# gue-ni/raytracer.c

Hardware: AMD Instinct MI355X
Metric: ray-bounces/sec (higher is better)
Workload: dtype f64

## Files before the change

raytracer.c_amd/csrc/pt_body_pooled.h:

```cpp
#ifndef PT_BODY_POOLED_H
#define PT_BODY_POOLED_H


#ifndef PT_MIN_WAVES
#define PT_MIN_WAVES 5
#endif
#ifndef PT_MIN_WAVES_TRI
#define PT_MIN_WAVES_TRI 5
#endif
#ifndef PT_MIN_WAVES_CHK
#define PT_MIN_WAVES_CHK 5
#endif
#ifndef PT_MESH_BATCH
#define PT_MESH_BATCH 32
#endif
#ifndef PT_MESH_MAX_WAIT
#define PT_MESH_MAX_WAIT 16
#endif
#ifndef PT_DIR_ROUNDS
#define PT_DIR_ROUNDS 4
#endif
#ifndef PT_DIR_MIN_LANES
#define PT_DIR_MIN_LANES 1
#endif
template <bool CHECKER, bool TRIS, bool FILT_LDS, bool GEOM_LDS, bool REFR = false>
__device__ __forceinline__ void render_tiles_pooled(const PtLaunch &L, const bool LIST)
{
  static_assert(!REFR || (CHECKER && FILT_LDS && (GEOM_LDS || !TRIS)), "the pooled refraction kernels: sphere scenes (staged, or streamed from memory) and small staged mesh scenes, every material");
  extern __shared__ __attribute__((aligned(16))) double lds[];
  __shared__ float out_f[PT_TILE_PIXELS * 3];
  __shared__ uint8_t out_b[PT_TILE_PIXELS * 3 + 64];
  __shared__ unsigned long long wg_stats[2];
  __shared__ double cam_lds[PT_CAM_LDS_DOUBLES];
  __shared__ unsigned long long pix_sum[REFR ? 1 : PT_TILE_PIXELS * 3];
  __shared__ unsigned long long pix_win[REFR ? PT_TILE_PIXELS * 3 * PT_WIN_N : 1];
  __shared__ unsigned long long pend_free[REFR ? PT_BLOCK / 64 : 1][2];
  __shared__ uint32_t pend_slot_lds;
  __shared__ unsigned long long pix_nan[3];
  __shared__ unsigned long long pix_key[PT_TILE_PIXELS];
  constexpr bool DEFER_MESH = TRIS && !FILT_LDS;
  constexpr bool SWAP = !DEFER_MESH;
  __shared__ double q_dir[SWAP ? 1 : PT_BLOCK / 64][SWAP ? 1 : 3 * 64];
  __shared__ unsigned long long q_rng[SWAP ? 1 : PT_BLOCK / 64][SWAP ? 1 : 64];
  __shared__ uint32_t q_pix[SWAP ? 1 : PT_BLOCK / 64][SWAP ? 1 : 64];
  constexpr uint32_t WAIT_F = CHECKER ? 11u : 10u;
  __shared__ double w_f[SWAP ? PT_BLOCK / 64 : 1][SWAP ? WAIT_F : 1][SWAP ? 64 : 1];
  __shared__ uint32_t w_u[SWAP ? PT_BLOCK / 64 : 1][SWAP ? 2 : 1][SWAP ? 64 : 1];
  constexpr uint32_t CULL_WORDS = GEOM_LDS ? PT_FILT_LDS_MAX / 64 : 256u;
  __shared__ uint32_t tile_pairs[CULL_WORDS];
  __shared__ uint32_t wg_next_job;

#ifdef PT_PHASE
  if ((threadIdx.x & 63u) == 0u)
  {
    for (int k = 0; k < PT_PHASE_SLOTS; k++)
      pt_phase_acc[threadIdx.x >> 6][k] = 0;
    pt_phase_last[threadIdx.x >> 6] = __builtin_amdgcn_s_memtime();
  }
#endif
  SceneCtx S_init = stage_scene<GEOM_LDS, FILT_LDS>(L, lds);
  __shared__ double atan_tab[CHECKER ? PT_ATAN_TAB : 1];
  if (CHECKER)
  {
    atan_table_to_lds(atan_tab);
    S_init.atan_tab = atan_tab;
  }
  PHASE(8);
  __shared__ __attribute__((aligned(16))) float big_tab[12];
  if (SWAP && FILT_LDS && !TRIS && L.big_pairs != 0u)
  {
    if (threadIdx.x < 2 + 2 * PT_BIG_PAIRS)
      big_tab[threadIdx.x] = threadIdx.x == 0 ? L.big_delta : (threadIdx.x == 1 ? L.big_tmin : L.big_qmin[threadIdx.x - 2]);
    S_init.big = BigPrune{big_tab, L.big_pairs};
  }
  const SceneCtx S = S_init;
  if (threadIdx.x < 2)
    wg_stats[threadIdx.x] = 0;
  if (threadIdx.x == 2)
    wg_next_job = 0;
  if (threadIdx.x < 3)
    pix_nan[threadIdx.x] = 0;
  if (!REFR && threadIdx.x < PT_TILE_PIXELS * 3)
    pix_sum[threadIdx.x] = 0;
  if (REFR)
  {
    for (uint32_t k = threadIdx.x; k < PT_TILE_PIXELS * 3 * PT_WIN_N; k += PT_BLOCK)
      pix_win[k] = 0;
    if (threadIdx.x < 2 * (PT_BLOCK / 64))
      pend_free[threadIdx.x >> 1][threadIdx.x & 1u] = ~0ull;
    if (threadIdx.x == 0)
      pend_slot_lds = pt_pool_acquire(L.pend_flags, L.pend_slots_per_xcd, L.status, PT_FAIL_PEND_SLOT);
  }
  if (threadIdx.x < PT_TILE_PIXELS)
  {
    const uint32_t t0 = L.tile_first + launch_slot(L, blockIdx.x % launch_slots(L, LIST), LIST) * L.tile_stride;
    const uint32_t kx = (t0 % L.tiles_x) * PT_TILE + (threadIdx.x & 7u), ky = (t0 / L.tiles_x) * PT_TILE + (threadIdx.x >> 3);
    pix_key[threadIdx.x] = rt_rng_pixel_key(L.seed, ky * (uint32_t)L.width + kx);
  }
  camera_to_lds(L, cam_lds);
  PHASE(9);
  __syncthreads();
  PHASE(10);

  const uint32_t wave = threadIdx.x >> 6;
  const uint32_t slot = launch_slot(L, blockIdx.x % launch_slots(L, LIST), LIST), chunk = blockIdx.x / launch_slots(L, LIST);
  const uint32_t tile = L.tile_first + slot * L.tile_stride;
  const bool cull_ok = S.n_sph + S.n_tri <= 64u * CULL_WORDS;
  if (SWAP && FILT_LDS && cull_ok)
  {
    tile_cull(cam_lds, L.scene.entry_src, S.n_sph, S.n_sph + S.n_tri, (tile % L.tiles_x) * PT_TILE, (tile / L.tiles_x) * PT_TILE, tile_pairs);
    __syncthreads();
  }
  const uint32_t tx0 = (tile % L.tiles_x) * PT_TILE, ty0 = (tile / L.tiles_x) * PT_TILE + (SWAP ? 0u : 2u * wave);
  const uint32_t vcols = min((uint32_t)PT_TILE, (uint32_t)L.width - tx0);
  const uint32_t vrows = ty0 >= (uint32_t)L.height ? 0u : min(SWAP ? (uint32_t)PT_TILE : 2u, (uint32_t)L.height - ty0);
  const uint32_t n_valid = vcols * vrows;
  const uint32_t spp = (uint32_t)L.samples;
  const uint32_t s_begin = L.sample_first + (uint32_t)(((uint64_t)chunk * spp) / L.sample_chunks);
  const uint32_t s_end = L.sample_first + (uint32_t)(((uint64_t)(chunk + 1u) * spp) / L.sample_chunks);
  const uint32_t pool_jobs = n_valid * (s_end - s_begin);

  Path P;
  P.o = {0, 0, 0};
  P.d = {0, 0, 1};
  P.T = {1, 1, 1};
  P.Ls = {0, 0, 0};
  P.rng = 1;
  P.depth = 0;
  uint32_t n_rays = 0, n_casts = 0;
  constexpr bool PARK_T = TRIS && FILT_LDS && !CHECKER;
  __shared__ double t_park[PARK_T ? 3 : 1][PARK_T ? PT_BLOCK : 1];
  HitRec hit;
  hit.min_t = 0;
  hit.bary_u = 0;
  hit.bary_v = 0;
  hit.best = -1;
  hit.depth_ok = false;
  hit.need_dir = false;
  hit.dir_slot = 0;
  hit.dir_scale = 1.0;
  hit.last.idx = -1;
  hit.last.u = 0;
  hit.last.v = 0;
  bool mesh_wait = false;
  uint32_t trip = 0, wait_since = 0xFFFFFFFFu;
  uint32_t next_job = 0;
  uint32_t made_jobs = 0;
  uint32_t pix_slot = 0;
  bool busy = false;
  int stack_n = 0;
  uint32_t pend_id = 0xFFu;
  const PendStack no_stack = {nullptr, 0, 0u, 0u};
  const uint32_t pend_slot = REFR ? pend_slot_lds : 0u;
  const bool pend_ok = !REFR || pend_slot != 0xFFFFFFFFu;
  const uint32_t pool = pend_ok ? pool_jobs : 0u;
  double *const pend_wave = REFR && pend_ok ? L.pend_ws + (size_t)pend_slot * L.pend_slot_doubles +
                                                  (size_t)(threadIdx.x >> 6) * 128u * L.pend_entries * PT_PEND_FIELDS
                                            : nullptr;
  unsigned long long *diag_ptr = L.stats;
  (void)diag_ptr;
  const uint32_t lane = threadIdx.x & 63u;
  double *const qd = q_dir[wave];
  unsigned long long *const qr = q_rng[wave];
  uint32_t *const qp = q_pix[wave];

  uint32_t n_wait = 0;
  double *const wf = &w_f[SWAP ? wave : 0][0][0];
  uint32_t *const wu = &w_u[SWAP ? wave : 0][0][0];
  PHASE(11);
  for (;;)
  {
    bool primary_trip = false;
    if (SWAP)
    {
      unsigned long long idle = __ballot(!busy);
      if (idle != 0 && n_wait != 0u)
      {
        const uint32_t rank = __builtin_amdgcn_mbcnt_hi((uint32_t)(idle >> 32), __builtin_amdgcn_mbcnt_lo((uint32_t)idle, 0u));
        if (!busy && rank < n_wait)
        {
          const uint32_t e = n_wait - 1u - rank;
          P.o = {wf[0 * 64 + e], wf[1 * 64 + e], wf[2 * 64 + e]};
          P.d = {wf[3 * 64 + e], wf[4 * 64 + e], wf[5 * 64 + e]};
          P.T = {wf[6 * 64 + e], wf[7 * 64 + e], wf[8 * 64 + e]};
          P.rng = (uint64_t)__double_as_longlong(wf[9 * 64 + e]);
          if (CHECKER)
            hit.dir_scale = wf[(CHECKER ? 10 : 0) * 64 + e];
          const uint32_t meta = wu[e];
          hit.dir_slot = wu[64 + e];
          pix_slot = meta & 63u;
          hit.need_dir = (meta & 64u) != 0u;
          P.depth = (int)((meta >> 7) & 63u);
          if (REFR)
          {
            stack_n = (int)((meta >> 13) & 63u);
            pend_id = (meta >> 19) & 0xFFu;
          }
          else
            P.depth = (int)(meta >> 7);
          busy = true;
        }
        n_wait -= min((uint32_t)__popcll(idle), n_wait);
        __builtin_amdgcn_fence(__ATOMIC_ACQUIRE, "wavefront");
        __builtin_amdgcn_wave_barrier();
        idle = __ballot(!busy);
      }
      PHASE(6);
      uint32_t batch = 0;
      if (idle != 0 && next_job < pool)
      {
        if (lane == 0)
          batch = atomicAdd(&wg_next_job, 64u);
        batch = (uint32_t)__builtin_amdgcn_readfirstlane((int)batch);
        next_job = batch < pool ? 0u : pool;
      }
      if (idle != 0 && next_job < pool)
      {
        const unsigned long long bm = __ballot(busy);
        if (busy)
        {
          const uint32_t e = __builtin_amdgcn_mbcnt_hi((uint32_t)(bm >> 32), __builtin_amdgcn_mbcnt_lo((uint32_t)bm, 0u));
          wf[0 * 64 + e] = P.o.x; wf[1 * 64 + e] = P.o.y; wf[2 * 64 + e] = P.o.z;
          wf[3 * 64 + e] = P.d.x; wf[4 * 64 + e] = P.d.y; wf[5 * 64 + e] = P.d.z;
          wf[6 * 64 + e] = P.T.x; wf[7 * 64 + e] = P.T.y; wf[8 * 64 + e] = P.T.z;
          wf[9 * 64 + e] = __longlong_as_double((long long)P.rng);
          if (CHECKER)
            wf[(CHECKER ? 10 : 0) * 64 + e] = hit.dir_scale;
          wu[e] = ((uint32_t)P.depth << 7) | (hit.need_dir ? 64u : 0u) | pix_slot |
                  (REFR ? (((uint32_t)stack_n << 13) | (pend_id << 19)) : 0u);
          wu[64 + e] = hit.dir_slot;
        }
        n_wait = (uint32_t)__popcll(bm);
        __builtin_amdgcn_fence(__ATOMIC_RELEASE, "wavefront");
        __builtin_amdgcn_wave_barrier();
        PHASE(7);
        const uint32_t job = batch + lane;
        busy = job < pool;
        if (busy)
        {
          DIAG(6, 1);
          DIAG_LANES(7);
          uint32_t idx;
          uint64_t term;
          if (n_valid == PT_TILE_PIXELS)
          {
            idx = job & 63u;
            term = sample_term_uniform(s_begin + (job >> 6));
          }
          else
          {
            const uint32_t s = job / n_valid;
            idx = job - s * n_valid;
            term = sample_term(s_begin + s);
          }
          const uint32_t row = (vcols == PT_TILE) ? (idx >> 3) : (idx / vcols);
          const uint32_t col = idx - __umul24(row, vcols);
          pix_slot = row * PT_TILE + col;
          start_sample(P, load_camera_lds(cam_lds), pix_key[pix_slot], tx0 + col, ty0 + row, term);
          hit.need_dir = false;
          if (REFR)
          {
            stack_n = 0;
            pend_id = 0xFFu;
          }
        }
        primary_trip = FILT_LDS;
      }
    }
    else
    {
      unsigned long long idle = __ballot(!busy);
      while (idle != 0 && next_job < pool)
      {
        if (next_job == made_jobs)
        {
          const uint32_t job = made_jobs + lane;
          if (job < pool)
          {
            DIAG(6, 1);
            DIAG_LANES(7);
            uint32_t idx, s;
            if (n_valid == 16)
            {
              idx = job & 15u;
              s = job >> 4;
            }
            else
            {
              s = job / n_valid;
              idx = job - s * n_valid;
            }
            const uint32_t row = (vcols == PT_TILE) ? (idx >> 3) : (idx / vcols);
            const uint32_t col = idx - __umul24(row, vcols);
            const uint32_t slot_in_tile = (2u * wave + row) * PT_TILE + col;
            Path Q;
            start_sample(Q, load_camera_lds(cam_lds), pix_key[slot_in_tile], tx0 + col, ty0 + row, sample_term(s_begin + s));
            qd[lane] = Q.d.x;
            qd[64 + lane] = Q.d.y;
            qd[128 + lane] = Q.d.z;
            qr[lane] = Q.rng;
            qp[lane] = slot_in_tile;
          }
          made_jobs = min(made_jobs + 64u, pool);
          __builtin_amdgcn_fence(__ATOMIC_RELEASE, "wavefront");
          __builtin_amdgcn_wave_barrier();
        }
        const uint32_t rank = __builtin_amdgcn_mbcnt_hi((uint32_t)(idle >> 32), __builtin_amdgcn_mbcnt_lo((uint32_t)idle, 0u));
        const uint32_t job = next_job + rank;
        if (!busy && job < made_jobs)
        {
          const uint32_t q = job & 63u;
          P.o = load_camera_pos_lds(cam_lds);
          P.d = {qd[q], qd[64 + q], qd[128 + q]};
          P.rng = qr[q];
          pix_slot = qp[q];
          P.T = {1, 1, 1};
          P.Ls = {0, 0, 0};
          P.depth = 0;
          busy = true;
        }
        next_job = min(next_job + (uint32_t)__popcll(idle), made_jobs);
        __builtin_amdgcn_fence(__ATOMIC_ACQUIRE, "wavefront");
        __builtin_amdgcn_wave_barrier();
        idle = __ballot(!busy);
      }
    }
    if (__ballot(busy) == 0)
      break;
    const uint32_t *const prim_pairs = (SWAP && FILT_LDS && primary_trip && cull_ok) ? tile_pairs : nullptr;
    PHASE(0);

    bool step_done = false;
    const bool stepping = busy && !hit.need_dir;
    if (DEFER_MESH)
    {
      if (stepping && !mesh_wait)
      {
        DIAG(0, 1);
        DIAG_LANES(1);
        n_rays++;
        (void)trace_step<1, false, CHECKER, TRIS, FILT_LDS, 1, true>(S, P, n_casts, diag_ptr, no_stack, stack_n, &hit);
        const bool far_origin = !(v_dot(P.o, P.o) <= S.near_R2);
        mesh_wait = hit.depth_ok && bvh_probe(S.bvh_nodes, S.n_bvh_nodes, far_origin, P.o, P.d,
                                              (CHECKER && S.stale_uv) ? S.t_start : hit.min_t, S.mesh_bound);
      }
      const uint32_t n_wait = (uint32_t)__popcll(__ballot(busy && mesh_wait));
      const uint32_t n_go = (uint32_t)__popcll(__ballot(busy && !mesh_wait));
      if (n_wait != 0 && wait_since == 0xFFFFFFFFu)
        wait_since = trip;
      const bool walk = n_wait != 0 && (n_wait >= PT_MESH_BATCH || n_go == 0 || trip - wait_since >= PT_MESH_MAX_WAIT);
      if (walk)
      {
        if (busy && mesh_wait)
        {
          const bool far_origin = !(v_dot(P.o, P.o) <= S.near_R2);
          bvh_traverse<CHECKER>(S.bvh_nodes, S.n_bvh_nodes, S.bvh_tri, S.tri, S.n_sph, far_origin, P.o, P.d, hit.min_t,
                                hit.best, hit.bary_u, hit.bary_v, diag_ptr, &hit.last, S.stale_uv, nullptr, S.tri32);
          mesh_wait = false;
        }
        wait_since = 0xFFFFFFFFu;
      }
      trip++;
      if (stepping && !mesh_wait)
        step_done = trace_step<1, false, CHECKER, TRIS, FILT_LDS, 2, true>(S, P, n_casts, diag_ptr, no_stack, stack_n, &hit);
    }
    else if (PARK_T)
    {
      if (stepping)
      {
        DIAG(0, 1);
        DIAG_LANES(1);
        n_rays++;
        t_park[0][threadIdx.x] = P.T.x;
        t_park[1][threadIdx.x] = P.T.y;
        t_park[2][threadIdx.x] = P.T.z;
        asm volatile("" ::: "memory");
        (void)trace_step<1, false, CHECKER, TRIS, FILT_LDS, 1, true>(S, P, n_casts, diag_ptr, no_stack, stack_n, &hit, prim_pairs);
        asm volatile("" ::: "memory");
        P.T = {t_park[0][threadIdx.x], t_park[1][threadIdx.x], t_park[2][threadIdx.x]};
        step_done = trace_step<1, false, CHECKER, TRIS, FILT_LDS, 2, true>(S, P, n_casts, diag_ptr, no_stack, stack_n, &hit);
      }
    }
    else if (stepping)
    {
      DIAG(0, 1);
      DIAG_LANES(1);
      n_rays++;
      if (REFR)
      {
        const PoolStack mine = {pend_wave, pend_free[wave], &pend_id, (int)L.pend_entries};
        step_done = trace_step<1, true, CHECKER, TRIS, FILT_LDS, 0, true, false, FILT_LDS && !GEOM_LDS, PoolStack>(S, P, n_casts, diag_ptr, mine, stack_n, &hit, prim_pairs);
      }
      else
        step_done = trace_step<1, false, CHECKER, TRIS, FILT_LDS, 0, true, false, FILT_LDS && !GEOM_LDS>(S, P, n_casts, diag_ptr, no_stack, stack_n, &hit, prim_pairs);
    }
    PHASE(3);
    if (busy && hit.need_dir)
    {
      V3 q;
      double len2;
      bool again = true;
      for (int round = 0; round < PT_DIR_ROUNDS && again; round++)
      {
        DIAG(10, 1);
        DIAG_LANES(11);
        again = rejection_round(P.rng, q, len2);
#if PT_DIR_MIN_LANES > 1
        if (__popcll(__ballot(again)) < PT_DIR_MIN_LANES)
          break;
#endif
      }
      if (!again)
      {
        const double *m = S.mat + PT_MAT_STRIDE * (hit.dir_slot & ~PT_HULL_PLUS);
        V3 albedo = ld3(m + 1);
        if (CHECKER)
          albedo = v_scale(albedo, hit.dir_scale);
        const V3 n = P.d;
        double weight;
        P.d = hemisphere_from_sample(q, len2, n, weight);
        P.T = v_mul(P.T, v_scale(albedo, weight));
        hit.need_dir = false;
      }
    }
    PHASE(4);
    if (busy)
    {
      if ((int)(P.Ls.x != 0.0) | (int)(P.Ls.y != 0.0) | (int)(P.Ls.z != 0.0))
      {
        if (REFR)
        {
          unsigned long long *const pw = &pix_win[__umul24(pix_slot, 3u * PT_WIN_N)];
          if (P.Ls.x != 0.0 && !win_add(pw, P.Ls.x)) atomicOr(&pix_nan[0], 1ull << pix_slot);
          if (P.Ls.y != 0.0 && !win_add(pw + PT_WIN_N, P.Ls.y)) atomicOr(&pix_nan[1], 1ull << pix_slot);
          if (P.Ls.z != 0.0 && !win_add(pw + 2 * PT_WIN_N, P.Ls.z)) atomicOr(&pix_nan[2], 1ull << pix_slot);
        }
        else
        {
        unsigned long long *const px = &pix_sum[__umul24(pix_slot, 3u)];
        atomicAdd(&px[0], fixed_term(P.Ls.x, L.acc_scale));
        atomicAdd(&px[1], fixed_term(P.Ls.y, L.acc_scale));
        atomicAdd(&px[2], fixed_term(P.Ls.z, L.acc_scale));
        if ((int)(P.Ls.x != P.Ls.x) | (int)(P.Ls.y != P.Ls.y) | (int)(P.Ls.z != P.Ls.z))
        {
          if (P.Ls.x != P.Ls.x) atomicOr(&pix_nan[0], 1ull << pix_slot);
          if (P.Ls.y != P.Ls.y) atomicOr(&pix_nan[1], 1ull << pix_slot);
          if (P.Ls.z != P.Ls.z) atomicOr(&pix_nan[2], 1ull << pix_slot);
        }
        }
      }
      if (step_done)
      {
        busy = false;
        if (REFR && pend_id != 0xFFu)
        {
          pend_id_give(pend_free[wave], pend_id);
          pend_id = 0xFFu;
        }
      }
    }
    P.Ls = {0, 0, 0};
    PHASE(5);
  }

  if (n_rays)
  {
    atomicAdd(&wg_stats[0], (unsigned long long)n_rays);
    atomicAdd(&wg_stats[1], (unsigned long long)n_casts);
  }
  __syncthreads();
  PHASE(12);

  if (REFR)
  {
    if (!pend_ok && threadIdx.x < 3)
      pix_nan[threadIdx.x] = ~0ull;
    __syncthreads();
    if (L.sample_chunks == 1 && !L.acc_keep)
    {
      if (threadIdx.x < PT_TILE_PIXELS * 3)
      {
        const uint32_t t = threadIdx.x / 3u, c = threadIdx.x - 3u * t;
        const bool inside = (tile % L.tiles_x) * PT_TILE + (t & 7u) < (uint32_t)L.width && (tile / L.tiles_x) * PT_TILE + (t >> 3) < (uint32_t)L.height;
        win_normalize(&pix_win[threadIdx.x * PT_WIN_N]);
        double mean = win_value(&pix_win[threadIdx.x * PT_WIN_N]) * (1.0 / (double)L.samples);
        mean = ((pix_nan[c] >> t) & 1ull) ? __longlong_as_double(0x7FF8000000000000ll) : mean;
        out_f[threadIdx.x] = inside ? (float)mean : 0.f;
        out_b[threadIdx.x] = inside ? tonemap(mean) : 0;
      }
      __syncthreads();
      store_tile(L, out_f, out_b, wg_stats, tile, slot, S.n_sph + S.n_tri, true, true);
    }
    else
    {
      if (threadIdx.x < PT_TILE_PIXELS * 3)
      {
        unsigned long long *const w = &pix_win[threadIdx.x * PT_WIN_N];
        win_normalize(w);
        unsigned long long *const acc = L.acc_ws + ((size_t)slot * (PT_TILE_PIXELS * 3) + threadIdx.x) * PT_WIN_N;
#pragma unroll
        for (int k = 0; k < PT_WIN_N; k++)
          if (w[k] != 0ull)
            atomicAdd(&acc[k], w[k]);
      }
      if (threadIdx.x < 3 && pix_nan[threadIdx.x] != 0)
        atomicOr(&L.acc_ws[(size_t)L.tile_count * (PT_TILE_PIXELS * 3 * PT_WIN_N) + (size_t)slot * 3 + threadIdx.x], pix_nan[threadIdx.x]);
      store_tile(L, out_f, out_b, wg_stats, tile, slot, S.n_sph + S.n_tri, false, chunk == 0);
    }
    if (pend_ok && threadIdx.x == 0)
      atomicExch(&L.pend_flags[pend_slot], 0u);
  }
  else if (L.sample_chunks == 1 && !L.acc_keep)
  {
    finish_pixels(L, pix_sum, pix_nan, tile, out_f, out_b);
    __syncthreads();
    store_tile(L, out_f, out_b, wg_stats, tile, slot, S.n_sph + S.n_tri, true, true);
    PHASE(13);
#ifdef PT_PHASE
    if ((threadIdx.x & 63u) == 0u && L.stats && (blockIdx.x & 31u) == 0u)
      for (int k = 0; k < PT_PHASE_SLOTS; k++)
        atomicAdd(&L.stats[64 + k], pt_phase_acc[threadIdx.x >> 6][k]);
#endif
  }
  else
  {
    if (threadIdx.x < PT_TILE_PIXELS * 3 && pix_sum[threadIdx.x] != 0)
      atomicAdd(&L.acc_ws[(size_t)slot * (PT_TILE_PIXELS * 3) + threadIdx.x], pix_sum[threadIdx.x]);
    if (threadIdx.x < 3 && pix_nan[threadIdx.x] != 0)
      atomicOr(&L.acc_ws[(size_t)L.tile_count * (PT_TILE_PIXELS * 3) + (size_t)slot * 3 + threadIdx.x], pix_nan[threadIdx.x]);
    store_tile(L, out_f, out_b, wg_stats, tile, slot, S.n_sph + S.n_tri, false, chunk == 0);
  }
}

#endif
```

raytracer.c_amd/csrc/rt_hip_shim.hip:

```cpp
#include <hip/hip_runtime.h>
#include <rccl/rccl.h>

#include <algorithm>
#include <atomic>
#include <chrono>
#include <cmath>
#include <cstdarg>
#include <cstdio>
#include <cstdlib>
#include <cstring>
#include <limits>
#include <mutex>
#include <new>
#include <utility>
#include <vector>

#include "pt_device.h"
#include "rt_hip.h"
#include "bvh_build.h"

static_assert(sizeof(RtHipSphere) == 88, "RtHipSphere must match the reference Object");
static_assert(sizeof(RtHipVertex) == 40, "RtHipVertex must match the reference Vertex");
static_assert(sizeof(RtHipCamera) == 96, "RtHipCamera must match the reference Camera");
static_assert(RT_HIP_TILE == PT_TILE && RT_HIP_TILE_PIXELS == PT_TILE_PIXELS, "tile shape");
// ... 779 lines not shown
  bool mesh_round = false;
  if (n_tri != 0)
  {
    double lo[3] = {HUGE_VAL, HUGE_VAL, HUGE_VAL}, hi[3] = {-HUGE_VAL, -HUGE_VAL, -HUGE_VAL};
    auto corner = [&](size_t tri, int k, double *p) {
      const double *g = &tgeom[9 * tri];
      for (int a = 0; a < 3; a++)
        p[a] = k == 0 ? g[a] : g[a] + g[3 * k + a];
    };
    for (size_t i = 0; i < n_tri; i++)
      for (int k = 0; k < 3; k++)
      {
        double p[3];
        corner(i, k, p);
        for (int a = 0; a < 3; a++)
        {
          lo[a] = std::fmin(lo[a], p[a]);
          hi[a] = std::fmax(hi[a], p[a]);
        }
      }
    for (int a = 0; a < 3; a++)
      mesh_c[a] = 0.5 * lo[a] + 0.5 * hi[a];
    double r2 = 0;
    for (size_t i = 0; i < n_tri; i++)
      for (int k = 0; k < 3; k++)
      {
        double p[3];
        corner(i, k, p);
        const double dx = p[0] - mesh_c[0], dy = p[1] - mesh_c[1], dz = p[2] - mesh_c[2];
        r2 = std::fmax(r2, dx * dx + dy * dy + dz * dz);
      }
    mesh_R = std::sqrt(r2) * (1.0 + 1e-9) + 1e-300;
    if (!(mesh_R < HUGE_VAL))
      mesh_R = HUGE_VAL;
    const double a = hi[0] - lo[0], b = hi[1] - lo[1], c = hi[2] - lo[2];
    mesh_round = 3.14159265358979 * mesh_R * mesh_R <= 0.5 * (a * b + b * c + c * a);
  }

  BvhBuild bvh;
  if (n_tri > 0)
  {
    bvh.tgeom = tgeom.data();
    bvh.order.resize(n_tri);
    bvh.cen.resize(3 * n_tri);
    bvh.lo.resize(3 * n_tri);
    bvh.hi.resize(3 * n_tri);
    for (uint32_t k = 0; k < (uint32_t)n_tri; k++)
    {
      bvh.order[k] = k;
      bvh.tri_box(k);
    }
    if (n_tri >= (1u << (31 - PT_BVH_COUNT_BITS)))
      return fail(RT_HIP_ELIMIT, "%zu triangles exceed the hierarchy's leaf references (2^%d)", n_tri, 31 - PT_BVH_COUNT_BITS);
    bvh.build_root((uint32_t)n_tri);
    if (bvh.depth > PT_BVH_STACK)
      return fail(RT_HIP_ELIMIT, "triangle hierarchy depth %d exceeds the traversal stack (%d)", bvh.depth, PT_BVH_STACK);
  }
  const size_t n_bvh_nodes = bvh.nodes.size() / PT_BVH_SRC_DOUBLES;
  std::vector<double> tgeom_leaf(9 * bvh.order.size());
  for (size_t k = 0; k < bvh.order.size(); k++)
    memcpy(&tgeom_leaf[9 * k], &tgeom[9 * (size_t)bvh.order[k]], 9 * sizeof(double));

  auto pad = [](size_t b) { return (b + 255) & ~(size_t)255; };
  const size_t off_geom = 0;
  const size_t off_mat = off_geom + pad(geom.size() * 8);
  const size_t off_craw = off_mat + pad(mat.size() * 8);
  const size_t off_geom4 = off_craw + pad(craw.size() * 8);
  const size_t off_tgeom = off_geom4 + pad(geom4.size() * 8);
  const size_t off_tnorm = off_tgeom + pad(tgeom.size() * 8);
  const size_t off_ttex = off_tnorm + pad(tnorm.size() * 8);
  const size_t off_tobj = off_ttex + pad(ttex.size() * 8);
  const size_t off_filt = off_tobj + pad(tobj.size() * 4);
  const size_t filt_bytes = pt_filt_bytes((uint32_t)n_spheres, (uint32_t)n_tri);
  const size_t off_bvh_src = off_filt + pad(filt_bytes);
  const size_t off_bvh_nodes = off_bvh_src + pad(bvh.nodes.size() * 8);
  const size_t bvh_nodes_bytes = n_bvh_nodes * PT_BVH_NODE_WORDS * 4;
  const size_t off_bvh_tri = off_bvh_nodes + pad(bvh_nodes_bytes);
  const size_t off_tgeom_leaf = off_bvh_tri + pad(bvh.order.size() * 4);
  const size_t total = off_tgeom_leaf + pad(tgeom_leaf.size() * 8) + 256;

  DeviceScope scope(device);
  HIP_TRY(scope.status);
  RtHipScene *sc = new (std::nothrow) RtHipScene;
  if (!sc)
    return fail(RT_HIP_ENOMEM, "host allocation failed");
  sc->device = device;
  hipError_t e = hipMalloc(&sc->blob, total);
  if (e != hipSuccess)
  {
    delete sc;
    return fail(RT_HIP_ENOMEM, "hipMalloc(%zu): %s", total, hipGetErrorString(e));
  }
  char *base = static_cast<char *>(sc->blob);
  auto up = [&](size_t off, const void *src, size_t bytes) -> hipError_t {
    return bytes ? hipMemcpy(base + off, src, bytes, hipMemcpyHostToDevice) : hipSuccess;
  };
  e = up(off_geom, geom.data(), geom.size() * 8);
  if (e == hipSuccess) e = up(off_mat, mat.data(), mat.size() * 8);
  if (e == hipSuccess) e = up(off_craw, craw.data(), craw.size() * 8);
  if (e == hipSuccess) e = up(off_geom4, geom4.data(), geom4.size() * 8);
  if (e == hipSuccess) e = up(off_tgeom, tgeom.data(), tgeom.size() * 8);
  if (e == hipSuccess) e = up(off_tnorm, tnorm.data(), tnorm.size() * 8);
  if (e == hipSuccess) e = up(off_ttex, ttex.data(), ttex.size() * 8);
  if (e == hipSuccess) e = up(off_tobj, tobj.data(), tobj.size() * 4);
  if (e == hipSuccess) e = up(off_bvh_src, bvh.nodes.data(), bvh.nodes.size() * 8);
  if (e == hipSuccess) e = up(off_bvh_tri, bvh.order.data(), bvh.order.size() * 4);
  if (e == hipSuccess) e = up(off_tgeom_leaf, tgeom_leaf.data(), tgeom_leaf.size() * 8);
  if (e != hipSuccess)
  {
    (void)hipFree(sc->blob);
    delete sc;
    return fail(RT_HIP_ERUNTIME, "scene upload: %s", hipGetErrorString(e));
  }
  sc->view.entry_src = reinterpret_cast<const double *>(base + off_geom);
  sc->view.filt = reinterpret_cast<float *>(base + off_filt);
  sc->view.bvh_src = reinterpret_cast<const double *>(base + off_bvh_src);
  sc->view.bvh_nodes = reinterpret_cast<float *>(base + off_bvh_nodes);
  sc->view.bvh_tri = reinterpret_cast<const uint32_t *>(base + off_bvh_tri);
  sc->view.tri_geom_leaf = reinterpret_cast<const double *>(base + off_tgeom_leaf);
  sc->view.n_bvh_nodes = (uint32_t)n_bvh_nodes;
  sc->view.bvh_depth = (uint32_t)bvh.depth;
  for (int a = 0; a < 3; a++)
    sc->mesh_c[a] = mesh_c[a];
  sc->mesh_R = mesh_R;
  sc->mesh_c_norm = std::sqrt(mesh_c[0] * mesh_c[0] + mesh_c[1] * mesh_c[1] + mesh_c[2] * mesh_c[2]) * (1.0 + 1e-12);
  sc->filt_bytes = filt_bytes;
  sc->bvh_nodes_bytes = bvh_nodes_bytes;
  sc->view.material = reinterpret_cast<const double *>(base + off_mat);
  sc->view.color_raw = reinterpret_cast<const double *>(base + off_craw);
  sc->view.geom4 = reinterpret_cast<const double *>(base + off_geom4);
  sc->view.tri_geom = reinterpret_cast<const double *>(base + off_tgeom);
  sc->view.tri_normal = reinterpret_cast<const double *>(base + off_tnorm);
  sc->view.tri_tex = reinterpret_cast<const double *>(base + off_ttex);
  sc->view.tri_object = reinterpret_cast<const uint32_t *>(base + off_tobj);
  if (n_tri != 0 && n_tri <= PT_HULL_MAX_TRIS && mesh_R >= 0 && mesh_R < 1e150)
  {
    const double extent = sc->mesh_c_norm + mesh_R;
    hipError_t he = pt_launch_build_hull_flags(sc->view.tri_geom, sc->view.tri_normal, (uint32_t)n_tri,
                                               1.1368683772161603e-13 * extent, reinterpret_cast<uint32_t *>(base + off_tobj), nullptr);
    if (he == hipSuccess)
      he = hipDeviceSynchronize();
    if (he != hipSuccess)
    {
      (void)hipFree(sc->blob);
      delete sc;
      return fail(RT_HIP_ERUNTIME, "hull flags: %s", hipGetErrorString(he));
    }
    sc->hull_flags = true;
  }
  sc->view.n_spheres = (uint32_t)n_spheres;
  sc->view.n_meshes = (uint32_t)n_meshes;
  sc->view.n_triangles = (uint32_t)n_tri;
  sc->view.any_checker = any_checker ? 1u : 0u;
  sc->view.mesh_round = mesh_round ? 1u : 0u;
  sc->view.any_refract = any_refract ? 1u : 0u;
#ifdef PT_DEV_KERNELS
  {
    const char *fb = getenv("RT_HIP_FORCE_BIG");
    if (fb && fb[0] == '1')
      wide_range = true;
  }
#endif
  sc->view.wide_range = wide_range ? 1u : 0u;
  sc->max_center = max_center;
  {
    int nb = 0;
    while (nb < 8 && (size_t)nb < n_spheres && std::fabs(spheres[nb].radius) >= 1000.0 && std::fabs(spheres[nb].radius) <= 1e17)
    {
      sc->big_r[nb] = std::fabs(spheres[nb].radius);
      sc->big_c[nb] = geom[PT_ENTRY_SRC_STRIDE * (size_t)nb + 4];
      nb++;
    }
    sc->n_big = nb & ~1;
  }
  sc->reach = reach;
  sc->max_emission = max_emission;
  sc->any_mirror_glass = any_mirror_glass;
  sc->view.any_mirror_glass = any_mirror_glass ? 1u : 0u;
  *out_scene = sc;
  return RT_HIP_OK;
}

bool park_ws_expected(const RtHipScene *scene)
{
  std::lock_guard<std::mutex> lock(scene->table_mutex);
  return scene->park_tried ? scene->park_ws != nullptr : (g_fail_alloc.load() & RT_HIP_FAIL_ALLOC_PARK_WS) == 0;
}

void mesh_bound_for(const RtHipScene *scene, double near_R, float out[5])
{
  const float inf = std::numeric_limits<float>::infinity();
  out[0] = out[1] = out[2] = 0.f;
  out[3] = inf;
  out[4] = -inf;
  if (!(scene->mesh_R >= 0) || !(scene->mesh_R < 1e18) || !(scene->mesh_c_norm < 1e18) || !(near_R < 1e18))
    return;
  const double e = 5.9604644775390625e-08, A = scene->mesh_c_norm + near_R;
  for (int a = 0; a < 3; a++)
    out[a] = (float)scene->mesh_c[a];
  out[3] = (float)((scene->mesh_R * scene->mesh_R + 32.0 * e * A * A) * (1.0 + 8.0 * e));
  out[4] = -(float)((scene->mesh_R + 10.0 * e * A) * (1.0 + 4.0 * e));
}

void big_prune_for(const RtHipScene *scene, double near_R, double filt_shift, PtLaunch &L)
{
  L.big_pairs = 0;
  L.big_delta = L.big_tmin = 0.f;
  for (int k = 0; k < 8; k++)
    L.big_qmin[k] = std::numeric_limits<float>::infinity();
#ifdef PT_DEV_KERNELS
  static const bool off = [] {
    const char *e = getenv("RT_HIP_NO_BIG_PRUNE");
    return e && e[0] == '1';
  }();
#else
  const bool off = false;
#endif
  const bool sign_form = !scene->view.wide_range &&
                         (pt_geom_in_lds(scene->view) ? (scene->view.n_triangles == 0 ? pt_filter_in_lds(scene->view) : !pt_filter_in_lds(scene->view))
                                                      : (scene->view.n_triangles == 0));
  if (off || scene->n_big < 2 || !sign_form)
    return;
  const double e = 5.9604644775390625e-08, f = 1.0 / 16.0;
  double delta = 0, tmin = 0;
  for (int k = 0; k < scene->n_big; k++)
  {
    const double r = scene->big_r[k], c = scene->big_c[k], A = c + near_R + filt_shift;
    const double g = std::fabs(c * c - r * r);
    const double W = pt_sign_widen_total(A, g) * 1.001, E = 28.0 * e * A * A + 6.0 * e * g;
    const double qmin = f * f * r * r + W + E;
    const double bias = (W + E) / (2.0 * f * r);
    if (!(qmin < 1e30) || !(bias < 1e3))
      return;
    L.big_qmin[k] = (float)(qmin * (1.0 + 4.0 * e));
    delta = std::fmax(delta, 1.5 * (22.4 * e * A + bias));
    tmin = std::fmax(tmin, 2.0 * (filt_shift * 1.0001 + 11.2 * e * A));
  }
  L.big_delta = (float)(delta * (1.0 + 4.0 * e));
  L.big_tmin = (float)(tmin * (1.0 + 4.0 * e));
  L.big_pairs = (uint32_t)scene->n_big / 2u;
}

double hull_margin_for(const RtHipScene *scene, double near_R)
{
  if (!scene->hull_flags || !(near_R < 1e150))
    return 2.0;
  const double extent = scene->mesh_c_norm + scene->mesh_R;
  const double tau = 1.1368683772161603e-13 * extent, delta = 1.4e-13 * (near_R + extent);
  return std::fmax(1e-3, 4.0 * (tau + delta) / 1e-8);
}

int launch_prepare(const RtHipScene *scene, const RtHipCamera *camera, const RtHipParams *params, PtLaunch &L, bool *empty)
{
  const int rc = check_params(params);
  if (rc)
    return rc;
  const bool cast_ray = params->integrator == RT_HIP_CAST_RAY;
  if (!cast_ray && scene->view.any_refract && params->max_depth > PT_REFRACT_MAX_DEPTH)
    return fail(RT_HIP_ELIMIT, "scenes with M_REFRACTION materials support max_depth <= %d (two rays per "
                               "refractive hit, raytracer.c:523-529; the pending-ray stack is fixed)",
                PT_REFRACT_MAX_DEPTH);
  if (cast_ray && scene->any_mirror_glass && params->max_depth > PT_REFRACT_MAX_DEPTH)
    return fail(RT_HIP_ELIMIT, "cast_ray with M_REFLECTION|M_REFRACTION materials supports max_depth <= %d (two "
                               "rays per such hit, raytracer.c:609-628; the pending-ray stack is fixed)",
                PT_REFRACT_MAX_DEPTH);
  const uint32_t tx = tiles_x_of(params->width), ty = tiles_y_of(params->height);
  const uint64_t n_tiles = (uint64_t)tx * ty;
  *empty = params->tile_count == 0;
  if (*empty)
    return RT_HIP_OK;
  if (params->tile_stride == 0 && params->tile_count > 1)
    return fail(RT_HIP_EINVAL, "tile_stride must be >= 1");
  const uint64_t last = (uint64_t)params->tile_first + (uint64_t)(params->tile_count - 1) * params->tile_stride;
  if (last >= n_tiles)
    return fail(RT_HIP_EINVAL, "tile range [%u + k*%u, k < %u] exceeds the image's %llu tiles", params->tile_first,
                params->tile_stride, params->tile_count, (unsigned long long)n_tiles);

  memset(&L, 0, sizeof L);
  L.scene = scene->view;
  memcpy(L.cam.pos, camera->position, sizeof L.cam.pos);
  memcpy(L.cam.horizontal, camera->horizontal, sizeof L.cam.horizontal);
  memcpy(L.cam.vertical, camera->vertical, sizeof L.cam.vertical);
  memcpy(L.cam.llc, camera->lower_left_corner, sizeof L.cam.llc);
  L.width = params->width;
  L.height = params->height;
  L.samples = params->samples;
  L.max_depth = params->max_depth;
  L.seed = params->seed;
  {
    const double *c = camera->position;
    const double cam = std::sqrt(c[0] * c[0] + c[1] * c[1] + c[2] * c[2]);
    L.near_R = 1.5 * (cam + scene->reach) + 1.0;
    if (!(L.near_R < RT_NEAR_R_LIMIT))
      return fail(RT_HIP_EINVAL, "scene extent %g is not a usable finite bound", L.near_R);
    L.near_R2 = L.near_R * L.near_R;
    L.filt_shift = 12.0 * 5.9604644775390625e-08 * (scene->max_center + L.near_R) * (1.0 + 1e-9);
    mesh_bound_for(scene, L.near_R, L.mesh_bound);
    big_prune_for(scene, L.near_R, L.filt_shift, L);
    L.hull_margin = hull_margin_for(scene, L.near_R);
#ifdef PT_DIAG
    {
      const char *flag = getenv("RT_HIP_DIAG_WALK_REJECTED");
      L.diag_flags = (flag && flag[0] == '1') ? 1u : 0u;
    }
#endif
    L.background = 10 / 255.0;
    L.t_start = 1.7976931348623157e308;
    L.w_minus_1 = (double)params->width - 1.0;
    L.h_minus_1 = (double)params->height - 1.0;
    L.inv_w_minus_1 = 1.0 / L.w_minus_1;
    L.inv_h_minus_1 = 1.0 / L.h_minus_1;
  }
  {
    const int s = pt_acc_scale_exp(scene->max_emission, params->samples, params->max_depth);
    if (s == INT32_MIN)
      return fail(RT_HIP_EINVAL, "emission magnitudes give no finite radiance bound (%g)", scene->max_emission);
    L.acc_scale = std::ldexp(1.0, s);
    L.acc_inv_scale = std::ldexp(1.0, -s);
  }
  L.tile_first = params->tile_first;
  L.tile_stride = params->tile_stride;
  L.tile_count = params->tile_count;
  L.tiles_x = tx;
  L.integrator = cast_ray ? 1u : 0u;
  return RT_HIP_OK;
}

int launch_device_state(const RtHipScene *scene, PtLaunch &L)
{
  const bool cast_ray = L.integrator == 1u;
  const int rc = status_word_for(scene->device, &L.status);
  if (rc)
    return rc;
  if (scene->view.n_bvh_nodes != 0 && !cast_ray)
  {
    std::lock_guard<std::mutex> lock(scene->table_mutex);
    if (!scene->park_tried)
    {
      scene->park_tried = true;
      scene->park_ws = park_acquire_ws(scene->device, &scene->park_slots_per_xcd);
    }
    if (scene->park_ws)
    {
      L.park_flags = reinterpret_cast<uint32_t *>(scene->park_ws);
      L.park_ws = scene->park_ws + park_flag_bytes(scene->park_slots_per_xcd);
      L.park_slots_per_xcd = scene->park_slots_per_xcd;
    }
  }
  return RT_HIP_OK;
}

PtPlanAsk ask_for(const RtHipScene *scene, uint32_t integrator, int32_t samples, int32_t max_depth, uint32_t sample_chunks,
                  bool have_chunk_ws, uint32_t tile_count, bool have_park_ws)
{
  return {.integrator = integrator, .samples = samples, .max_depth = max_depth, .max_emission = scene->max_emission,
          .sample_chunks = sample_chunks, .have_chunk_ws = have_chunk_ws, .tile_count = tile_count, .have_park_ws = have_park_ws,
          .wide_pend_ok = true};
}

template <class PoolFn>
int plan_launch(const RtHipScene *scene, PtLaunch &L, uint32_t sample_chunks, bool have_chunk_ws, PoolFn take_pool, PtPlan *out)
{
  PtPlanAsk ask = ask_for(scene, L.integrator, L.samples, L.max_depth, sample_chunks, have_chunk_ws, L.tile_count, L.park_ws != nullptr);
  PtPlan plan = pt_plan_launch(L.scene, ask);
  int rc = plan.pend_entries ? take_pool(plan.pend_entries, plan.pend_columns, L) : RT_HIP_OK;
  if (rc == RT_HIP_ENOMEM && plan.pend_columns > PT_PEND_COLUMNS)
  {
    ask.wide_pend_ok = false;
    plan = pt_plan_launch(L.scene, ask);
    rc = plan.pend_entries ? take_pool(plan.pend_entries, plan.pend_columns, L) : RT_HIP_OK;
  }
  L.sample_chunks = plan.sample_chunks;
  L.acc_windows = plan.windowed ? 1u : 0u;
  *out = plan;
  return rc;
}

void accum_free(RtHipAccum *a)
{
  if (!a)
    return;
  DeviceScope scope(a->scene->device);
  (void)hipDeviceSynchronize();
  delete a;
}

int accum_adapt_state(RtHipAccum *a)
{
  if (a->tile_samples)
    return RT_HIP_OK;
  const size_t n = a->L.tile_count;
  const size_t bytes = (2 * n + 1) * sizeof(uint32_t) + n;
  DeviceBuffer buf;
  const hipError_t e = buf.alloc(bytes);
  if (e != hipSuccess)
    return fail(RT_HIP_ENOMEM, "freeze state (%zu KB): %s", bytes >> 10, hipGetErrorString(e));
  HIP_TRY(hipMemset(buf.ptr, 0, bytes));
  HIP_TRY(hipStreamSynchronize(nullptr));
  a->tile_samples = std::move(buf);
  a->slot_list = a->tile_samples.at<uint32_t>() + n;
  a->d_live_count = a->slot_list + n;
  a->keep = reinterpret_cast<uint8_t *>(a->d_live_count + 1);
  a->live_count = (uint32_t)n;
  return RT_HIP_OK;
}

int accum_freeze(RtHipAccum *a, const float *d_error, const uint8_t *h_keep, double threshold, uint32_t dilate, uint32_t *live_count,
                        void *stream)
{
  if (live_count)
    *live_count = 0;
  if (!a)
    return fail(RT_HIP_EINVAL, "accumulation is NULL");
  if (!d_error && !h_keep)
    return fail(RT_HIP_EINVAL, "a freeze needs the tile errors or a keep mask");
  if (dilate > 2u)
    return fail(RT_HIP_EINVAL, "dilate is 0 .. 2 tiles, not %u", dilate);
  if (a->done < 1)
    return fail(RT_HIP_EINVAL, "the accumulation holds no sample yet");
  if (a->broken)
    return fail(RT_HIP_ERUNTIME, "the accumulation is unusable: an earlier freeze failed on the device");
  const PtLaunch &L = a->L;
  if (d_error && !(threshold > 0.0))
  {
    if (live_count)
      *live_count = a->tile_samples ? a->live_count : L.tile_count;
    return RT_HIP_OK;
  }
  DeviceScope scope(a->scene->device);
  HIP_TRY(scope.status);
  int rc = accum_adapt_state(a);
  if (rc)
    return rc;
  hipStream_t st = static_cast<hipStream_t>(stream);
  hipError_t e = hipSuccess;
  if (!d_error)
    e = hipMemcpyAsync(a->keep, h_keep, L.tile_count, hipMemcpyHostToDevice, st);
  if (e == hipSuccess)
    e = pt_launch_tile_freeze(d_error, threshold, (int)dilate, a->keep, a->tile_samples.at<uint32_t>(), L.width, L.height, L.tile_first, L.tile_stride,
                              L.tile_count, (uint32_t)a->done, a->slot_list, a->d_live_count, st);
  uint32_t n = 0;
  if (e == hipSuccess)
    e = hipMemcpyAsync(&n, a->d_live_count, sizeof n, hipMemcpyDeviceToHost, st);
  if (e == hipSuccess)
    e = hipStreamSynchronize(st);
  if (e != hipSuccess)
  {
    a->broken = true;
    return fail(RT_HIP_ERUNTIME, "freeze: %s", hipGetErrorString(e));
  }
  a->live_count = n;
  a->any_frozen = a->any_frozen || n < L.tile_count;
  if (live_count)
    *live_count = n;
  return RT_HIP_OK;
}

int adaptive_passes(RtHipAccum *a, const RtHipAdaptParams *p, uint64_t *h_stats,
                    int (*on_checkpoint)(void *user, int32_t samples_done, uint32_t live_tiles), void *user, double *seconds)
{
  const PtLaunch &L = a->L;
  const size_t tile_vals = (size_t)L.tile_count * PT_TILE_PIXELS * 3;
  const bool estimate = p->threshold > 0.0;
  if (estimate && !a->adapt_buf)
  {
    const hipError_t e = a->adapt_buf.alloc((2 * tile_vals + L.tile_count) * sizeof(float));
    if (e != hipSuccess)
      return fail(RT_HIP_ENOMEM, "adaptive buffers: %s", hipGetErrorString(e));
  }
  float *prev = a->adapt_buf.at<float>(), *cur = prev + tile_vals, *err = prev + 2 * tile_vals;
  int32_t targets[32];
  const int n_targets = rt_hip_adapt_schedule(a->budget, p->min_samples, targets, 32);
  EventPair timer;
  HIP_TRY(timer.create());
  for (int i = 0; i < n_targets; i++)
  {
    if (targets[i] > a->done)
    {
      double pass_seconds = 0;
      const int rc = rt_hip_accum_add_host(a, targets[i] - a->done, h_stats, &pass_seconds);
      *seconds += pass_seconds;
      if (rc)
        return rc;
    }
    if (targets[i] == a->budget)
      break;
    uint32_t live = rt_hip_accum_live_tiles(a);
    if (estimate)
    {
      HIP_TRY(timer.start(nullptr));
      int rc = rt_hip_accum_resolve(a, i == 0 ? prev : cur, nullptr, nullptr);
      if (i > 0 && !rc)
      {
        rc = rt_hip_tile_error(cur, prev, L.width, L.height, L.tile_first, L.tile_stride, L.tile_count, err, nullptr);
        if (!rc)
          rc = rt_hip_accum_freeze(a, err, p->threshold, p->dilate, &live, nullptr);
        std::swap(prev, cur);
      }
      if (rc)
        return rc;
      HIP_TRY(timer.stop(nullptr));
      HIP_TRY(timer.wait());
      float ms = 0.f;
      HIP_TRY(timer.elapsed_ms(&ms));
      *seconds += 1e-3 * (double)ms;
    }
    if (i > 0 && on_checkpoint && on_checkpoint(user, a->done, live))
      return fail(RT_HIP_ECANCELLED, "adaptive render cancelled at %d samples", a->done);
    if (i > 0 && live == 0u)
      break;
  }
  return RT_HIP_OK;
}

bool aov_any(const RtHipAov *a) { return a && (a->albedo || a->normal || a->depth || a->object || a->hits); }

constexpr size_t TILE_VALS = (size_t)PT_TILE_PIXELS * 3;

struct ImageCtx
{
  struct Dev
  {
    RtHipScene *scene = nullptr;
    hipStream_t stream = nullptr;
    EventPair timer;
    hipEvent_t done = nullptr;
    DeviceBuffer tiles, tiles8, stats, ws;
    uint32_t count = 0;
    size_t first_slot = 0;
  };
  int G = 0, W = 0, H = 0;
  std::vector<int> phys, comm_of, lead;
  int n_phys = 0;
  bool force_comm = false;
  std::vector<unsigned char> scene_bytes;
  std::vector<Dev> dev;
  std::vector<ncclComm_t> comms;
  DeviceBuffer all_tiles, all_tiles8, image, image8;
  uint64_t builds = 0;
};
ImageCtx &g_ctx = *new ImageCtx;
std::mutex g_ctx_mutex;
double g_last_phases[3] = {0, 0, 0};

std::vector<int> g_device_map;
bool g_device_map_env_read = false;

void device_map_from_env()
{
  if (g_device_map_env_read)
    return;
  g_device_map_env_read = true;
  const char *e = getenv("RT_HIP_DEVICE_MAP");
  if (!e || !*e || !g_device_map.empty())
    return;
  std::vector<int> m;
  for (const char *p = e; *p;)
  {
    char *end = nullptr;
    const long v = strtol(p, &end, 10);
    if (end == p || v < 0 || v > 63)
      return;
    m.push_back((int)v);
    p = end;
    if (*p == ',')
      p++;
    else if (*p)
      return;
  }
  g_device_map = m;
}

void ctx_release(ImageCtx &c)
{
  int prev = 0;
  (void)hipGetDevice(&prev);
  for (int g = 0; g < (int)c.dev.size(); g++)
    if (c.dev[g].stream)
    {
      (void)hipSetDevice(c.phys[g]);
      (void)hipStreamSynchronize(c.dev[g].stream);
    }
  for (int r = 0; r < (int)c.comms.size(); r++)
    if (c.comms[r])
    {
      for (int g = 0; g < (int)c.comm_of.size(); g++)
        if (c.comm_of[g] == r)
        {
          (void)hipSetDevice(c.phys[g]);
          break;
        }
      (void)ncclCommDestroy(c.comms[r]);
    }
  for (int g = 0; g < (int)c.dev.size(); g++)
  {
    (void)hipSetDevice(c.phys[g]);
    ImageCtx::Dev &d = c.dev[g];
    if (d.done) (void)hipEventDestroy(d.done);
    if (d.stream) (void)hipStreamDestroy(d.stream);
    rt_hip_scene_destroy(d.scene);
    d = ImageCtx::Dev();
  }
  if (!c.phys.empty())
    (void)hipSetDevice(c.phys[0]);
  const uint64_t builds = c.builds;
  c = ImageCtx();
// ... 2575 lines not shown
```

Baseline: 45.59 billion.

## Park rays that fail rejection sampling in wave LDS and retry later

Lanes whose rejection-sampled direction is still unresolved after fewer rounds are parked into the top of the per-wave LDS swap buffer and freed. Idle lanes later pick them up again to retry. Radiance accumulation moves before the direction step so parked lanes retire cleanly. The goal is to cut divergence in the rejection loop, which keeps a whole wave spinning for a few lanes. The cost is extra LDS traffic and bookkeeping, and the swap buffer has to be shared with waiting mesh rays.

```diff
diff --git a/raytracer.c_amd/csrc/pt_body_pooled.h b/raytracer.c_amd/csrc/pt_body_pooled.h
--- a/raytracer.c_amd/csrc/pt_body_pooled.h
+++ b/raytracer.c_amd/csrc/pt_body_pooled.h
@@ -17,8 +17,14 @@
 #ifndef PT_MESH_MAX_WAIT
 #define PT_MESH_MAX_WAIT 16
 #endif
+#ifndef PT_DIR_PARK
+#define PT_DIR_PARK 1
+#endif
 #ifndef PT_DIR_ROUNDS
 #define PT_DIR_ROUNDS 4
+#endif
+#ifndef PT_DIR_PARK_ROUNDS
+#define PT_DIR_PARK_ROUNDS 2
 #endif
 #ifndef PT_DIR_MIN_LANES
 #define PT_DIR_MIN_LANES 1
@@ -165,6 +171,8 @@
   uint32_t *const qp = q_pix[wave];
 
   uint32_t n_wait = 0;
+  constexpr bool PARK = SWAP && PT_DIR_PARK != 0;
+  uint32_t n_retry = 0;
   double *const wf = &w_f[SWAP ? wave : 0][0][0];
   uint32_t *const wu = &w_u[SWAP ? wave : 0][0][0];
   PHASE(11);
@@ -207,14 +215,15 @@
       }
       PHASE(6);
       uint32_t batch = 0;
-      if (idle != 0 && next_job < pool)
+      const bool may_swap = idle != 0 && (!PARK || n_retry <= (uint32_t)__popcll(idle));
+      if (may_swap && next_job < pool)
       {
         if (lane == 0)
           batch = atomicAdd(&wg_next_job, 64u);
         batch = (uint32_t)__builtin_amdgcn_readfirstlane((int)batch);
         next_job = batch < pool ? 0u : pool;
       }
-      if (idle != 0 && next_job < pool)
+      if (may_swap && next_job < pool)
       {
         const unsigned long long bm = __ballot(busy);
         if (busy)
@@ -325,7 +334,7 @@
         idle = __ballot(!busy);
       }
     }
-    if (__ballot(busy) == 0)
+    if (__ballot(busy) == 0 && (!PARK || n_retry == 0u))
       break;
     const uint32_t *const prim_pairs = (SWAP && FILT_LDS && primary_trip && cull_ok) ? tile_pairs : nullptr;
     PHASE(0);
@@ -395,12 +404,89 @@
         step_done = trace_step<1, false, CHECKER, TRIS, FILT_LDS, 0, true, false, FILT_LDS && !GEOM_LDS>(S, P, n_casts, diag_ptr, no_stack, stack_n, &hit, prim_pairs);
     }
     PHASE(3);
+    const auto radiance_to_sums = [&]() {
+      if (busy)
+      {
+        if ((int)(P.Ls.x != 0.0) | (int)(P.Ls.y != 0.0) | (int)(P.Ls.z != 0.0))
+        {
+          if (REFR)
+          {
+            unsigned long long *const pw = &pix_win[__umul24(pix_slot, 3u * PT_WIN_N)];
+            if (P.Ls.x != 0.0 && !win_add(pw, P.Ls.x)) atomicOr(&pix_nan[0], 1ull << pix_slot);
+            if (P.Ls.y != 0.0 && !win_add(pw + PT_WIN_N, P.Ls.y)) atomicOr(&pix_nan[1], 1ull << pix_slot);
+            if (P.Ls.z != 0.0 && !win_add(pw + 2 * PT_WIN_N, P.Ls.z)) atomicOr(&pix_nan[2], 1ull << pix_slot);
+          }
+          else
+          {
+          unsigned long long *const px = &pix_sum[__umul24(pix_slot, 3u)];
+          atomicAdd(&px[0], fixed_term(P.Ls.x, L.acc_scale));
+          atomicAdd(&px[1], fixed_term(P.Ls.y, L.acc_scale));
+          atomicAdd(&px[2], fixed_term(P.Ls.z, L.acc_scale));
+          if ((int)(P.Ls.x != P.Ls.x) | (int)(P.Ls.y != P.Ls.y) | (int)(P.Ls.z != P.Ls.z))
+          {
+            if (P.Ls.x != P.Ls.x) atomicOr(&pix_nan[0], 1ull << pix_slot);
+            if (P.Ls.y != P.Ls.y) atomicOr(&pix_nan[1], 1ull << pix_slot);
+            if (P.Ls.z != P.Ls.z) atomicOr(&pix_nan[2], 1ull << pix_slot);
+          }
+          }
+        }
+        if (step_done)
+        {
+          busy = false;
+          if (REFR && pend_id != 0xFFu)
+          {
+            pend_id_give(pend_free[wave], pend_id);
+            pend_id = 0xFFu;
+          }
+        }
+      }
+    };
+    if (PARK)
+    {
+      radiance_to_sums();
+      PHASE(5);
+    }
+    constexpr int DIR_ROUNDS = PARK ? PT_DIR_PARK_ROUNDS : PT_DIR_ROUNDS;
+    if (PARK && n_retry != 0u)
+    {
+      const unsigned long long idle = __ballot(!busy);
+      if (idle != 0)
+      {
+        const uint32_t rank = __builtin_amdgcn_mbcnt_hi((uint32_t)(idle >> 32), __builtin_amdgcn_mbcnt_lo((uint32_t)idle, 0u));
+        if (!busy && rank < n_retry)
+        {
+          const uint32_t e = 64u - n_retry + rank;
+          P.o = {wf[0 * 64 + e], wf[1 * 64 + e], wf[2 * 64 + e]};
+          P.d = {wf[3 * 64 + e], wf[4 * 64 + e], wf[5 * 64 + e]};
+          P.T = {wf[6 * 64 + e], wf[7 * 64 + e], wf[8 * 64 + e]};
+          P.rng = (uint64_t)__double_as_longlong(wf[9 * 64 + e]);
+          if (CHECKER)
+            hit.dir_scale = wf[(CHECKER ? 10 : 0) * 64 + e];
+          const uint32_t meta = wu[e];
+          hit.dir_slot = wu[64 + e];
+          pix_slot = meta & 63u;
+          hit.need_dir = true;
+          if (REFR)
+          {
+            P.depth = (int)((meta >> 7) & 63u);
+            stack_n = (int)((meta >> 13) & 63u);
+            pend_id = (meta >> 19) & 0xFFu;
+          }
+          else
+            P.depth = (int)(meta >> 7);
+          busy = true;
+        }
+        n_retry -= min((uint32_t)__popcll(idle), n_retry);
+        __builtin_amdgcn_fence(__ATOMIC_ACQUIRE, "wavefront");
+        __builtin_amdgcn_wave_barrier();
+      }
+    }
     if (busy && hit.need_dir)
     {
       V3 q;
       double len2;
       bool again = true;
-      for (int round = 0; round < PT_DIR_ROUNDS && again; round++)
+      for (int round = 0; round < DIR_ROUNDS && again; round++)
       {
         DIAG(10, 1);
         DIAG_LANES(11);
@@ -423,42 +509,42 @@
         hit.need_dir = false;
       }
     }
+    if (PARK)
+    {
+      const unsigned long long pm = __ballot(busy && hit.need_dir);
+      if (pm != 0)
+      {
+        const uint32_t room = 64u - n_wait - n_retry, want = (uint32_t)__popcll(pm);
+        const uint32_t rank = __builtin_amdgcn_mbcnt_hi((uint32_t)(pm >> 32), __builtin_amdgcn_mbcnt_lo((uint32_t)pm, 0u));
+#ifdef PT_DIAG
+        if (L.diag_flags & 2u)
+        {
+          DIAG(44, min(want, room));
+          DIAG(45, want - min(want, room));
+        }
+#endif
+        if (busy && hit.need_dir && rank < room)
+        {
+          const uint32_t e = 63u - n_retry - rank;
+          wf[0 * 64 + e] = P.o.x; wf[1 * 64 + e] = P.o.y; wf[2 * 64 + e] = P.o.z;
+          wf[3 * 64 + e] = P.d.x; wf[4 * 64 + e] = P.d.y; wf[5 * 64 + e] = P.d.z;
+          wf[6 * 64 + e] = P.T.x; wf[7 * 64 + e] = P.T.y; wf[8 * 64 + e] = P.T.z;
+          wf[9 * 64 + e] = __longlong_as_double((long long)P.rng);
+          if (CHECKER)
+            wf[(CHECKER ? 10 : 0) * 64 + e] = hit.dir_scale;
+          wu[e] = ((uint32_t)P.depth << 7) | 64u | pix_slot | (REFR ? (((uint32_t)stack_n << 13) | (pend_id << 19)) : 0u);
+          wu[64 + e] = hit.dir_slot;
+          hit.need_dir = false;
+          busy = false;
+        }
+        n_retry += min(want, room);
+        __builtin_amdgcn_fence(__ATOMIC_RELEASE, "wavefront");
+        __builtin_amdgcn_wave_barrier();
+      }
+    }
     PHASE(4);
-    if (busy)
-    {
-      if ((int)(P.Ls.x != 0.0) | (int)(P.Ls.y != 0.0) | (int)(P.Ls.z != 0.0))
-      {
-        if (REFR)
-        {
-          unsigned long long *const pw = &pix_win[__umul24(pix_slot, 3u * PT_WIN_N)];
-          if (P.Ls.x != 0.0 && !win_add(pw, P.Ls.x)) atomicOr(&pix_nan[0], 1ull << pix_slot);
-          if (P.Ls.y != 0.0 && !win_add(pw + PT_WIN_N, P.Ls.y)) atomicOr(&pix_nan[1], 1ull << pix_slot);
-          if (P.Ls.z != 0.0 && !win_add(pw + 2 * PT_WIN_N, P.Ls.z)) atomicOr(&pix_nan[2], 1ull << pix_slot);
-        }
-        else
-        {
-        unsigned long long *const px = &pix_sum[__umul24(pix_slot, 3u)];
-        atomicAdd(&px[0], fixed_term(P.Ls.x, L.acc_scale));
-        atomicAdd(&px[1], fixed_term(P.Ls.y, L.acc_scale));
-        atomicAdd(&px[2], fixed_term(P.Ls.z, L.acc_scale));
-        if ((int)(P.Ls.x != P.Ls.x) | (int)(P.Ls.y != P.Ls.y) | (int)(P.Ls.z != P.Ls.z))
-        {
-          if (P.Ls.x != P.Ls.x) atomicOr(&pix_nan[0], 1ull << pix_slot);
-          if (P.Ls.y != P.Ls.y) atomicOr(&pix_nan[1], 1ull << pix_slot);
-          if (P.Ls.z != P.Ls.z) atomicOr(&pix_nan[2], 1ull << pix_slot);
-        }
-        }
-      }
-      if (step_done)
-      {
-        busy = false;
-        if (REFR && pend_id != 0xFFu)
-        {
-          pend_id_give(pend_free[wave], pend_id);
-          pend_id = 0xFFu;
-        }
-      }
-    }
+    if (!PARK)
+      radiance_to_sums();
     P.Ls = {0, 0, 0};
     PHASE(5);
   }
diff --git a/raytracer.c_amd/csrc/rt_hip_shim.hip b/raytracer.c_amd/csrc/rt_hip_shim.hip
--- a/raytracer.c_amd/csrc/rt_hip_shim.hip
+++ b/raytracer.c_amd/csrc/rt_hip_shim.hip
@@ -1105,6 +1105,8 @@
     {
       const char *flag = getenv("RT_HIP_DIAG_WALK_REJECTED");
       L.diag_flags = (flag && flag[0] == '1') ? 1u : 0u;
+      const char *park = getenv("RT_HIP_DIAG_PARK_COUNTS");
+      L.diag_flags |= (park && park[0] == '1') ? 2u : 0u;
     }
 #endif
     L.background = 10 / 255.0;
```

After: 46.62 billion, median of 6. 1.02x the previous value.
